# MalvinaNikandrou/mafed

Measured on AMD Instinct MI355X. Metric: train samples/sec VLPythia-410M+MAFED, 256img+32txt tok, bs=32, 1/2/4/8 GPU, higher is better.
Workload: dtype bf16; 1 GPU; VLPythia-410m + MAFED distill step (student fwd+bwd, frozen-teacher fwd, replay CE, 23-layer per-modality MSE, clip 2.0, AdamW), 256 img + 32 txt tokens; global_batch=32, per_gpu_batch=32, seq_len=288, parallelism=dp1, random_init_weights=True

## Files before the change

### mafed_amd/csrc/attn_mfma.hip

```cpp
#include <type_traits>

#include "attn.h"
#include "row8.h"

namespace mafed {

namespace {

typedef __attribute__((address_space(3))) bf16x4* lds_bf16x4_ptr;

template <int D>
__device__ __forceinline__ int swz(int row) {
  if (D == 64) return ((row >> 1) & 3) << 1;
  if (D == 128) return (row & 7) << 1;
  return ((row & 7) << 1) | ((row >> 3) & 1);
}
template <int D>
__device__ __forceinline__ int tile_off(int row, int chunk) {
  if (D == 64) return row * 128 + ((chunk ^ swz<64>(row)) << 4);
  if (D == 128) return row * 256 + ((chunk ^ swz<128>(row)) << 4);
  return row * 512 + ((chunk ^ (((row & 7) << 1) | ((row >> 3) & 1))) << 4);
}

__device__ __forceinline__ uint4 load_chunk_rot(const bf16_t* __restrict__ rowp, int chunk, int rot, const float* __restrict__ rc,
// ... 256 lines not shown
  const bf16_t* kb = qb + D;
  const bf16_t* vb = qb + 2 * D;
  const int q0 = qt * 64 + wave * 16;
  const int myq = q0 + (lane & 15);
  const int g = lane >> 4;

  bf16x8 qf[D / 32];
  load_col_frags<D, true>(qf, qb, rstride, q0, S, rot, rc, rs, lane);

  f32x4 o[D / 16];
#pragma unroll
  for (int i = 0; i < D / 16; ++i) o[i] = (f32x4){0.f, 0.f, 0.f, 0.f};
  float m = -INFINITY, l = 0.f;
  const float scale = rsqrtf((float)D);

  for (int kt = 0; kt <= qt; ++kt) {
    __syncthreads();
    stage_rows<D, 64, true>(kimg, kb, rstride, kt * 64, S, rot, rc, rs, tid);
    stage_rows<D, 64, false>(vimg, vb, rstride, kt * 64, S, rot, rc, rs, tid);
    __syncthreads();
    const bool need_mask = (kt == qt) || (kt * 64 + 63 >= P);
    fwd_tile_step<D>(kimg, vimg, qf, o, m, l, scale, need_mask, kt * 64, g, lane,
                     [&](int key) { return key > myq || !key_ok(am, b, key, P, T, S); });
  }
  l = col_sum(l);
  if (myq < S) {
    store_out<D>(out + ((int64_t)b * S + myq) * H * D + (int64_t)h * D, o, l, g);
    if (g == 0) lse[((int64_t)b * H + h) * S + myq] = m + logf(l);
  }
}

template <int D>
__global__ __launch_bounds__(256) void attn_suffix_mfma_kernel(const bf16_t* __restrict__ qkv_img, const int64_t* __restrict__ image_index,
                                                               const bf16_t* __restrict__ qkv_txt, SuffixShape sh, const float* __restrict__ rc,
                                                               const float* __restrict__ rs, const int64_t* __restrict__ am,
                                                               bf16_t* __restrict__ out) {
  extern __shared__ __attribute__((aligned(16))) char lds[];
  char* kimg = lds;
  char* vimg = lds + 64 * D * 2;
  const int tid = threadIdx.x, lane = tid & 63;
  const int wave = __builtin_amdgcn_readfirstlane(tid >> 6);
  const int P = sh.P, T = sh.T, S = sh.P + sh.T, H = sh.H, rot = sh.rot;
  const int qt = blockIdx.x, h = blockIdx.y, b = blockIdx.z;
  const int64_t rstride = (int64_t)H * 3 * D;
  const bf16_t* ib = qkv_img + (suffix_image(image_index, b, sh.N) * P * H + h) * 3 * D;
  const bf16_t* tb = qkv_txt + ((int64_t)b * T * H + h) * 3 * D;
  const int q0 = qt * 64 + wave * 16;
  const int myq = q0 + (lane & 15), mypos = P + myq;
  const int g = lane >> 4;
  const bool active = q0 < T;

  bf16x8 qf[D / 32];
#pragma unroll
  for (int ks = 0; ks < D / 32; ++ks)
    qf[ks] = __builtin_bit_cast(bf16x8, load_chunk_rot(tb + (int64_t)myq * rstride, ks * 4 + g, rot, rc, rs, mypos, myq < T));

  f32x4 o[D / 16];
#pragma unroll
  for (int i = 0; i < D / 16; ++i) o[i] = (f32x4){0.f, 0.f, 0.f, 0.f};
  float m = -INFINITY, l = 0.f;
  const float scale = rsqrtf((float)D);
  const int last_q = min(qt * 64 + 63, T - 1);
  const int nkt = (P + last_q) / 64 + 1;

  for (int kt = 0; kt < nkt; ++kt) {
    __syncthreads();
    const auto row = [&](int gr) { return StageRow{gr < P ? ib + (int64_t)gr * rstride : tb + (int64_t)(gr - P) * rstride, gr, gr < S}; };
    stage_rows_by<D, true>(kimg, tid, kt * 64, D, rot, rc, rs, row);
    stage_rows_by<D, false>(vimg, tid, kt * 64, 2 * D, rot, rc, rs, row);
    __syncthreads();
    if (!active || kt * 64 > P + q0 + 15) continue;
    const bool need_mask = kt * 64 + 63 >= P;
    fwd_tile_step<D>(kimg, vimg, qf, o, m, l, scale, need_mask, kt * 64, g, lane,
                     [&](int key) { return key > mypos || !key_ok(am, b, key, P, T, S); });
  }
  l = col_sum(l);
  if (myq < T) store_out<D>(out + ((int64_t)b * T + myq) * H * D + (int64_t)h * D, o, l, g);
}

template <int D>
__global__ __launch_bounds__(256) void attn_cand_mfma_kernel(const bf16_t* __restrict__ qkv_pre, const bf16_t* __restrict__ qkv_cand, CandShape sh,
                                                             const float* __restrict__ rc, const float* __restrict__ rs,
                                                             const int64_t* __restrict__ am, bf16_t* __restrict__ out) {
  extern __shared__ __attribute__((aligned(16))) char lds[];
  char* kimg = lds;
  char* vimg = lds + 64 * D * 2;
  const int tid = threadIdx.x, lane = tid & 63;
  const int wave = __builtin_amdgcn_readfirstlane(tid >> 6);
  const int S0 = sh.S0, T = sh.T, P = sh.S0 - sh.T, A = sh.A, CA = sh.C * sh.A, H = sh.H, rot = sh.rot;
  const int qt = blockIdx.x, h = blockIdx.y, b = blockIdx.z;
  const int64_t rstride = (int64_t)H * 3 * D;
  const bf16_t* pb = qkv_pre + ((int64_t)b * S0 * H + h) * 3 * D;
  const bf16_t* cb = qkv_cand + ((int64_t)b * CA * H + h) * 3 * D;
  const int q0 = qt * 64 + wave * 16;
  const int myq = q0 + (lane & 15);
  const int mystart = myq / A * A;
  const int g = lane >> 4;
  const bool active = q0 < CA;

  bf16x8 qf[D / 32];
#pragma unroll
  for (int ks = 0; ks < D / 32; ++ks)
    qf[ks] = __builtin_bit_cast(bf16x8, load_chunk_rot(cb + (int64_t)myq * rstride, ks * 4 + g, rot, rc, rs, S0 + myq % A, myq < CA));

  f32x4 o[D / 16];
#pragma unroll
  for (int i = 0; i < D / 16; ++i) o[i] = (f32x4){0.f, 0.f, 0.f, 0.f};
  float m = -INFINITY, l = 0.f;
  const float scale = rsqrtf((float)D);
  const int nkp = (S0 + 63) / 64;
  const int k0 = qt * 64 / A * A;
  const int nkc = (min(qt * 64 + 63, CA - 1) - k0) / 64 + 1;
  const int wlo = q0 / A * A, whi = q0 + 15;

  for (int kt = 0; kt < nkp + nkc; ++kt) {
    const bool pre = kt < nkp;
    const int t0 = pre ? kt * 64 : k0 + (kt - nkp) * 64;
    __syncthreads();
    if (pre) {
      stage_rows<D, 64, true>(kimg, pb + D, rstride, t0, S0, rot, rc, rs, tid);
      stage_rows<D, 64, false>(vimg, pb + 2 * D, rstride, t0, S0, rot, rc, rs, tid);
    } else {
      const auto row = [&](int gr) { return StageRow{cb + (int64_t)gr * rstride, S0 + gr % A, gr < CA}; };
      stage_rows_by<D, true>(kimg, tid, t0, D, rot, rc, rs, row);
      stage_rows_by<D, false>(vimg, tid, t0, 2 * D, rot, rc, rs, row);
    }
    __syncthreads();
    if (!active || (!pre && (t0 > whi || t0 + 63 < wlo))) continue;
    const bool need_mask = !pre || t0 + 63 >= P;
    fwd_tile_step<D>(kimg, vimg, qf, o, m, l, scale, need_mask, t0, g, lane,
                     [&](int key) { return pre ? !key_ok(am, b, key, P, T, S0) : (key < mystart || key > myq); });
  }
  l = col_sum(l);
  if (myq < CA) store_out<D>(out + ((int64_t)b * CA + myq) * H * D + (int64_t)h * D, o, l, g);
}

template <int D>
__global__ __launch_bounds__(256) void attn_bwd_dq_mfma_kernel(const bf16_t* __restrict__ qkv, const bf16_t* __restrict__ out,
                                                               const bf16_t* __restrict__ dout, const float* __restrict__ lse, AttnShape sh,
                                                               const float* __restrict__ rc, const float* __restrict__ rs,
                                                               const int64_t* __restrict__ am, bf16_t* __restrict__ dqkv,
                                                               float* __restrict__ delta) {
  extern __shared__ __attribute__((aligned(16))) char lds[];
  char* kimg = lds;
  char* vimg = lds + 64 * D * 2;
  const int tid = threadIdx.x, lane = tid & 63, wave = tid >> 6;
  const int S = sh.S, H = sh.H, rot = sh.rot, P = sh.P, T = sh.T;
  const int qt = (int)gridDim.x - 1 - (int)blockIdx.x, h = blockIdx.y, b = blockIdx.z;
  const int64_t rstride = (int64_t)H * 3 * D;
  const bf16_t* qb = qkv + ((int64_t)b * S * H + h) * 3 * D;
  const bf16_t* kb = qb + D;
  const bf16_t* vb = qb + 2 * D;
  const int q0 = qt * 64 + wave * 16;
  const int myq = q0 + (lane & 15);
  const int g = lane >> 4;
  const int64_t ostride = (int64_t)H * D;
  const bf16_t* ob = out + (int64_t)b * S * ostride + (int64_t)h * D;
  const bf16_t* dob = dout + (int64_t)b * S * ostride + (int64_t)h * D;

  bf16x8 qf[D / 32], dof[D / 32];
  load_col_frags<D, true>(qf, qb, rstride, q0, S, rot, rc, rs, lane);
  load_col_frags<D, false>(dof, dob, ostride, q0, S, 0, rc, rs, lane);
  float dl = 0.f;
  {
    bf16x8 of[D / 32];
    load_col_frags<D, false>(of, ob, ostride, q0, S, 0, rc, rs, lane);
#pragma unroll
    for (int ks = 0; ks < D / 32; ++ks)
#pragma unroll
      for (int e = 0; e < 8; ++e) dl += (float)dof[ks][e] * (float)of[ks][e];
    dl = col_sum(dl);
  }
  float L = 0.f;
  if (myq < S) {
    L = lse[((int64_t)b * H + h) * S + myq];
    if (g == 0) delta[((int64_t)b * H + h) * S + myq] = dl;
  }
  f32x4 dq[D / 16];
#pragma unroll
  for (int i = 0; i < D / 16; ++i) dq[i] = (f32x4){0.f, 0.f, 0.f, 0.f};
  const float scale = rsqrtf((float)D);

  for (int kt = 0; kt <= qt; ++kt) {
    __syncthreads();
    stage_rows<D, 64, true>(kimg, kb, rstride, kt * 64, S, rot, rc, rs, tid);
    stage_rows<D, 64, false>(vimg, vb, rstride, kt * 64, S, rot, rc, rs, tid);
    __syncthreads();
    const bool need_mask = (kt == qt) || (kt * 64 + 63 >= P);
    f32x4 ds[4];
#pragma unroll
    for (int j = 0; j < 4; ++j) {
      f32x4 s = (f32x4){0.f, 0.f, 0.f, 0.f}, dp = (f32x4){0.f, 0.f, 0.f, 0.f};
#pragma unroll
      for (int ks = 0; ks < D / 32; ++ks) {
        s = __builtin_amdgcn_mfma_f32_16x16x32_bf16(frag_row<D>(kimg, j, ks, lane), qf[ks], s, 0, 0, 0);
        dp = __builtin_amdgcn_mfma_f32_16x16x32_bf16(frag_row<D>(vimg, j, ks, lane), dof[ks], dp, 0, 0, 0);
      }
#pragma unroll
      for (int r = 0; r < 4; ++r) {
        float p = __expf(s[r] * scale - L);
        if (need_mask) {
          const int key = kt * 64 + j * 16 + 4 * g + r;
          if (key > myq || !key_ok(am, b, key, P, T, S)) p = 0.f;
        }
        ds[j][r] = p * (dp[r] - dl) * scale;
      }
    }
    const bf16x8 d0 = pack_acc(ds[0], ds[1]), d1 = pack_acc(ds[2], ds[3]);
#pragma unroll
    for (int dt = 0; dt < D / 16; ++dt) {
      dq[dt] = __builtin_amdgcn_mfma_f32_16x16x32_bf16(frag_tr<D>(kimg, dt, 0, lane), d0, dq[dt], 0, 0, 0);
      dq[dt] = __builtin_amdgcn_mfma_f32_16x16x32_bf16(frag_tr<D>(kimg, dt, 1, lane), d1, dq[dt], 0, 0, 0);
    }
  }
  bf16_t* dqp = dqkv + ((int64_t)b * S * H + h) * 3 * D + (int64_t)myq * rstride;
  store_grad_unrot<D>(dqp, dq, rot, rc, rs, myq, lane, myq < S);
}

template <int D>
__global__ __launch_bounds__(256) void attn_bwd_dkv_mfma_kernel(const bf16_t* __restrict__ qkv, const bf16_t* __restrict__ dout,
                                                                const float* __restrict__ lse, const float* __restrict__ delta, AttnShape sh,
                                                                const float* __restrict__ rc, const float* __restrict__ rs,
                                                                const int64_t* __restrict__ am, bf16_t* __restrict__ dqkv) {
  extern __shared__ __attribute__((aligned(16))) char lds[];
  char* qimg = lds;
  char* doimg = lds + 64 * D * 2;
  float* Ls = reinterpret_cast<float*>(lds + 2 * 64 * D * 2);
  float* dls = Ls + 64;
  const int tid = threadIdx.x, lane = tid & 63, wave = tid >> 6;
  const int S = sh.S, H = sh.H, rot = sh.rot, P = sh.P, T = sh.T;
  const int kt = blockIdx.x, h = blockIdx.y, b = blockIdx.z;
  const int nqt = (S + 63) / 64;
  const int64_t rstride = (int64_t)H * 3 * D;
  const bf16_t* qb = qkv + ((int64_t)b * S * H + h) * 3 * D;
  const bf16_t* kb = qb + D;
  const bf16_t* vb = qb + 2 * D;
  const int64_t ostride = (int64_t)H * D;
  const bf16_t* dob = dout + (int64_t)b * S * ostride + (int64_t)h * D;
  const int k0 = kt * 64 + wave * 16;
  const int mykey = k0 + (lane & 15);
  const int g = lane >> 4;
  const bool mykey_ok = key_ok(am, b, mykey, P, T, S);

  bf16x8 kf[D / 32], vf[D / 32];
  load_col_frags<D, true>(kf, kb, rstride, k0, S, rot, rc, rs, lane);
  load_col_frags<D, false>(vf, vb, rstride, k0, S, 0, rc, rs, lane);
  f32x4 dk[D / 16], dv[D / 16];
#pragma unroll
  for (int i = 0; i < D / 16; ++i) { dk[i] = (f32x4){0.f, 0.f, 0.f, 0.f}; dv[i] = (f32x4){0.f, 0.f, 0.f, 0.f}; }
  const float scale = rsqrtf((float)D);
  const int64_t lbase = ((int64_t)b * H + h) * S;

  for (int qt = kt; qt < nqt; ++qt) {
    __syncthreads();
    stage_rows<D, 64, true>(qimg, qb, rstride, qt * 64, S, rot, rc, rs, tid);
    stage_rows<D, 64, false>(doimg, dob, ostride, qt * 64, S, 0, rc, rs, tid);
    if (tid < 64) {
      const int q = qt * 64 + tid;
      Ls[tid] = q < S ? lse[lbase + q] : 0.f;
      dls[tid] = q < S ? delta[lbase + q] : 0.f;
    }
    __syncthreads();
    f32x4 p[4], ds[4];
#pragma unroll
    for (int j = 0; j < 4; ++j) {
      f32x4 s = (f32x4){0.f, 0.f, 0.f, 0.f}, dp = (f32x4){0.f, 0.f, 0.f, 0.f};
#pragma unroll
      for (int ks = 0; ks < D / 32; ++ks) {
        s = __builtin_amdgcn_mfma_f32_16x16x32_bf16(frag_row<D>(qimg, j, ks, lane), kf[ks], s, 0, 0, 0);
        dp = __builtin_amdgcn_mfma_f32_16x16x32_bf16(frag_row<D>(doimg, j, ks, lane), vf[ks], dp, 0, 0, 0);
      }
      const float4 Lq = *reinterpret_cast<const float4*>(Ls + j * 16 + 4 * g);
      const float4 Dq = *reinterpret_cast<const float4*>(dls + j * 16 + 4 * g);
      const float La[4] = {Lq.x, Lq.y, Lq.z, Lq.w}, Da[4] = {Dq.x, Dq.y, Dq.z, Dq.w};
#pragma unroll
      for (int r = 0; r < 4; ++r) {
        const int q = qt * 64 + j * 16 + 4 * g + r;
        float pv = __expf(s[r] * scale - La[r]);
        if (!mykey_ok || mykey > q || q >= S) pv = 0.f;
        p[j][r] = pv;
        ds[j][r] = pv * (dp[r] - Da[r]) * scale;
      }
    }
    const bf16x8 p0 = pack_acc(p[0], p[1]), p1 = pack_acc(p[2], p[3]);
    const bf16x8 d0 = pack_acc(ds[0], ds[1]), d1 = pack_acc(ds[2], ds[3]);
#pragma unroll
    for (int dt = 0; dt < D / 16; ++dt) {
      dv[dt] = __builtin_amdgcn_mfma_f32_16x16x32_bf16(frag_tr<D>(doimg, dt, 0, lane), p0, dv[dt], 0, 0, 0);
      dv[dt] = __builtin_amdgcn_mfma_f32_16x16x32_bf16(frag_tr<D>(doimg, dt, 1, lane), p1, dv[dt], 0, 0, 0);
      dk[dt] = __builtin_amdgcn_mfma_f32_16x16x32_bf16(frag_tr<D>(qimg, dt, 0, lane), d0, dk[dt], 0, 0, 0);
      dk[dt] = __builtin_amdgcn_mfma_f32_16x16x32_bf16(frag_tr<D>(qimg, dt, 1, lane), d1, dk[dt], 0, 0, 0);
    }
  }
  bf16_t* dkp = dqkv + ((int64_t)b * S * H + h) * 3 * D + (int64_t)mykey * rstride + D;
  store_grad_unrot<D>(dkp, dk, rot, rc, rs, mykey, lane, mykey < S);
  if (mykey < S) {
    bf16_t* dvp = dkp + D;
#pragma unroll
    for (int dt = 0; dt < D / 16; ++dt) store4(dvp + dt * 16 + 4 * g, make_float4(dv[dt][0], dv[dt][1], dv[dt][2], dv[dt][3]));
  }
}

typedef __attribute__((address_space(3))) void* lds_void_ptr;
typedef const __attribute__((address_space(1))) void* glb_void_ptr;
typedef unsigned u32x2 __attribute__((ext_vector_type(2)));

__device__ __forceinline__ float col_max_sw(float v) {
  u32x2 r = __builtin_amdgcn_permlane32_swap(__float_as_uint(v), __float_as_uint(v), false, false);
  v = fmaxf(__uint_as_float(r[0]), __uint_as_float(r[1]));
  r = __builtin_amdgcn_permlane16_swap(__float_as_uint(v), __float_as_uint(v), false, false);
  return fmaxf(__uint_as_float(r[0]), __uint_as_float(r[1]));
}
__device__ __forceinline__ float col_sum_sw(float v) {
  u32x2 r = __builtin_amdgcn_permlane32_swap(__float_as_uint(v), __float_as_uint(v), false, false);
  v = __uint_as_float(r[0]) + __uint_as_float(r[1]);
  r = __builtin_amdgcn_permlane16_swap(__float_as_uint(v), __float_as_uint(v), false, false);
  return __uint_as_float(r[0]) + __uint_as_float(r[1]);
}

template <int D, int NW = 4>
__device__ __forceinline__ void dma_rows(char* __restrict__ img, const bf16_t* __restrict__ base, int64_t rstride, int nrows, int S, int wave,
                                         int lane) {
  constexpr int RPP = 1024 / (2 * D);
  const int npieces = nrows / RPP;
  for (int j = wave; j < npieces; j += NW) {
    int row, logical;
    if (D == 64) {
      row = j * 8 + (lane >> 3);
      logical = (lane & 7) ^ swz<64>(row);
    } else {
      row = j * 4 + (lane >> 4);
      logical = (lane & 15) ^ swz<128>(row);
    }
    const int srow = row < S ? row : S - 1;
    __builtin_amdgcn_global_load_lds((glb_void_ptr)(base + (int64_t)srow * rstride + logical * 8), (lds_void_ptr)(img + j * 1024), 16, 0, 0);
  }
}

struct RotPre {
  float4 c0, c1, s0, s1;
};
__device__ __forceinline__ void rot_pre_load(RotPre& r, int it, int hc, int rot, const float* __restrict__ rc, const float* __restrict__ rs) {
  const int row = it / hc, c = it - row * hc;
  const float* cp = rc + (int64_t)row * (rot >> 1) + c * 8;
  const float* sp = rs + (int64_t)row * (rot >> 1) + c * 8;
  r.c0 = load4(cp); r.c1 = load4(cp + 4); r.s0 = load4(sp); r.s1 = load4(sp + 4);
}
template <int D>
__device__ __forceinline__ void rot_apply(char* __restrict__ img, int it, int hc, const RotPre& r) {
  const int row = it / hc, c = it - row * hc;
  uint4* p1 = reinterpret_cast<uint4*>(img + tile_off<D>(row, c));
  uint4* p2 = reinterpret_cast<uint4*>(img + tile_off<D>(row, c + hc));
  float x1[8], x2[8], o1[8], o2[8];
  unpack8(*p1, x1);
  unpack8(*p2, x2);
  const float cs[8] = {r.c0.x, r.c0.y, r.c0.z, r.c0.w, r.c1.x, r.c1.y, r.c1.z, r.c1.w};
  const float sn[8] = {r.s0.x, r.s0.y, r.s0.z, r.s0.w, r.s1.x, r.s1.y, r.s1.z, r.s1.w};
#pragma unroll
  for (int e = 0; e < 8; ++e) {
    o1[e] = x1[e] * cs[e] - x2[e] * sn[e];
    o2[e] = x2[e] * cs[e] + x1[e] * sn[e];
  }
  *p1 = pack8(o1);
  *p2 = pack8(o2);
}
template <int D, int NT = 256>
__device__ __forceinline__ void rot_fix_rows(char* __restrict__ img, int items, int hc, int rot, const float* __restrict__ rc,
                                             const float* __restrict__ rs, const RotPre (&pre)[2], int tid) {
#pragma unroll
  for (int u = 0; u < 2; ++u)
    if (tid + NT * u < items) rot_apply<D>(img, tid + NT * u, hc, pre[u]);
  for (int it = tid + 2 * NT; it < items; it += NT) {
    RotPre r;
    rot_pre_load(r, it, hc, rot, rc, rs);
    rot_apply<D>(img, it, hc, r);
  }
}

__device__ __forceinline__ float row16_sum(float v) {
  v += __builtin_bit_cast(float, __builtin_amdgcn_update_dpp(0, __builtin_bit_cast(int, v), 0xB1, 0xF, 0xF, true));
  v += __builtin_bit_cast(float, __builtin_amdgcn_update_dpp(0, __builtin_bit_cast(int, v), 0x4E, 0xF, 0xF, true));
  v += __builtin_bit_cast(float, __builtin_amdgcn_update_dpp(0, __builtin_bit_cast(int, v), 0x141, 0xF, 0xF, true));
  v += __builtin_bit_cast(float, __builtin_amdgcn_update_dpp(0, __builtin_bit_cast(int, v), 0x140, 0xF, 0xF, true));
  return v;
}

__device__ __forceinline__ void wait_vm0() { asm volatile("s_waitcnt vmcnt(0)" ::: "memory"); }

__device__ __forceinline__ int snake4(int w, int t) { return t * 4 + ((t & 1) ? 3 - w : w); }
template <int NW>
__device__ __forceinline__ int snake(int w, int t) { return t * NW + ((t & 1) ? NW - 1 - w : w); }

#define MAFED_LOG2E 1.4426950408889634f
#define MAFED_LN2 0.6931471805599453f

template <int D>
constexpr int attn_fwd_waves() { return D == 64 ? 8 : 4; }

template <int D, bool CAUSAL = true>
__global__ __launch_bounds__(attn_fwd_waves<D>() * 64, (D == 64 ? 2 : 1) * attn_fwd_waves<D>() / 4) void attn_fwd_res_kernel(const bf16_t* __restrict__ qkv, AttnShape sh, const float* __restrict__ rc,
                                                           const float* __restrict__ rs, const int64_t* __restrict__ am,
                                                           bf16_t* __restrict__ out, float* __restrict__ lse) {
  extern __shared__ __attribute__((aligned(16))) char lds[];
  constexpr int NW = attn_fwd_waves<D>(), NTH = NW * 64;
  const int tid = threadIdx.x, lane = tid & 63;
  const int wave = __builtin_amdgcn_readfirstlane(tid >> 6);
  const int S = sh.S, H = sh.H, rot = sh.rot, P = sh.P, T = sh.T;
  const int h = blockIdx.x, b = blockIdx.y;
  const int nrows = (S + 31) / 32 * 32;
  char* kimg = lds;
  char* vimg = lds + nrows * D * 2;
  float* kbias = reinterpret_cast<float*>(lds + 2 * nrows * D * 2);
  const int64_t rstride = (int64_t)H * 3 * D;
  const bf16_t* qb = qkv + ((int64_t)b * S * H + h) * 3 * D;
  const bf16_t* kb = qb + D;
  const bf16_t* vb = qb + 2 * D;
  const int nslices = (S + 15) / 16;
  const int hc = rot >> 4, items = S * hc;
#if defined(MAFED_ATTN_ABL) && MAFED_ATTN_ABL == 3
  if (tid == 0) out[((int64_t)b * S) * H * D + (int64_t)h * D] = 0;
  return;
#endif
  dma_rows<D, NW>(kimg, kb, rstride, nrows, S, wave, lane);
#if !defined(MAFED_ATTN_ABL) || MAFED_ATTN_ABL != 4
  dma_rows<D, NW>(vimg, vb, rstride, nrows, S, wave, lane);
#endif
  RotPre pre[2];
#pragma unroll
  for (int u = 0; u < 2; ++u)
    if (tid + NTH * u < items) rot_pre_load(pre[u], tid + NTH * u, hc, rot, rc, rs);
  for (int k = tid; k < nrows; k += NTH) kbias[k] = key_ok(am, b, k, P, T, S) ? 0.f : -INFINITY;
  ColRaw<D> qraw;
  {
    const int s0 = nslices - 1 - snake<NW>(wave, 0);
    if (s0 >= 0) col_raw_issue<D, true>(qraw, qb, rstride, s0 * 16, S, rot, rc, rs, lane);
  }
  wait_vm0();
  __syncthreads();
  rot_fix_rows<D, NTH>(kimg, items, hc, rot, rc, rs, pre, tid);
  __syncthreads();
#if defined(MAFED_ATTN_ABL) && (MAFED_ATTN_ABL == 1 || MAFED_ATTN_ABL == 4)
  if (tid < 64) out[((int64_t)b * S + tid) * H * D + (int64_t)h * D] = *reinterpret_cast<const bf16_t*>(kimg + tid * 1024) + *reinterpret_cast<const bf16_t*>(vimg + tid * 1024);
  return;
#endif
  const int g = lane >> 4;
  const float scale2 = rsqrtf((float)D) * MAFED_LOG2E;
  const bf16x8 ones = __builtin_bit_cast(bf16x8, make_uint4(0x3f803f80u, 0x3f803f80u, 0x3f803f80u, 0x3f803f80u));
  for (int t = 0;; ++t) {
    const int slice = nslices - 1 - snake<NW>(wave, t);
    if (slice < 0) break;
    const int q0 = slice * 16;
    const int myq = q0 + (lane & 15);
    bf16x8 qf[D / 32];
    col_raw_finish<D, true>(qf, qraw, q0, S, rot, lane);
    {
      const int nxt = nslices - 1 - snake<NW>(wave, t + 1);
      if (nxt >= 0) col_raw_issue<D, true>(qraw, qb, rstride, nxt * 16, S, rot, rc, rs, lane);
    }
    f32x4 o[D / 16];
#pragma unroll
    for (int i = 0; i < D / 16; ++i) o[i] = (f32x4){0.f, 0.f, 0.f, 0.f};
    float m = -INFINITY;
    f32x4 lsum = (f32x4){0.f, 0.f, 0.f, 0.f};
    const int last_kt = CAUSAL ? (q0 + 15) / 64 : (S - 1) / 64;
    auto tile = [&](const int kt, const int nj, auto mask_tag) {
      constexpr bool MASK = decltype(mask_tag)::value;
      f32x4 s[4];
#pragma unroll
      for (int j = 0; j < 4; ++j) {
        s[j] = (f32x4){0.f, 0.f, 0.f, 0.f};
        if (!MASK || j < nj) {
#pragma unroll
          for (int ks = 0; ks < D / 32; ++ks)
            s[j] = __builtin_amdgcn_mfma_f32_16x16x32_bf16(frag_row<D>(kimg, kt * 4 + j, ks, lane), qf[ks], s[j], 0, 0, 0);
        }
      }
      float tmax = -INFINITY;
      if (MASK) {
#pragma unroll
        for (int j = 0; j < 4; ++j) {
          if (j < nj) {
            const float4 kb4 = *reinterpret_cast<const float4*>(kbias + kt * 64 + j * 16 + 4 * g);
            const float kbv[4] = {kb4.x, kb4.y, kb4.z, kb4.w};
#pragma unroll
            for (int r = 0; r < 4; ++r) {
              const int key = kt * 64 + j * 16 + 4 * g + r;
              float v = s[j][r] * scale2 + kbv[r];
              if (CAUSAL) v = key > myq ? -INFINITY : v;
              s[j][r] = v;
              tmax = fmaxf(tmax, v);
            }
          } else {
            s[j] = (f32x4){-INFINITY, -INFINITY, -INFINITY, -INFINITY};
          }
        }
      } else {
#pragma unroll
        for (int j = 0; j < 4; ++j)
#pragma unroll
          for (int r = 0; r < 4; ++r) tmax = fmaxf(tmax, s[j][r]);
        tmax *= scale2;
      }
      tmax = col_max_sw(tmax);
      if (__builtin_amdgcn_ballot_w64(tmax - m > 8.0f) != 0) {
        const float mn = fmaxf(m, tmax);
        const float alpha = __builtin_amdgcn_exp2f(m - mn);
        m = mn;
        lsum *= alpha;
#pragma unroll
        for (int i = 0; i < D / 16; ++i) o[i] *= alpha;
      }
#pragma unroll
      for (int j = 0; j < 4; ++j)
#pragma unroll
        for (int r = 0; r < 4; ++r) s[j][r] = __builtin_amdgcn_exp2f(MASK ? s[j][r] - m : fmaf(s[j][r], scale2, -m));
      const bf16x8 p0 = pack_acc(s[0], s[1]);
      lsum = __builtin_amdgcn_mfma_f32_16x16x32_bf16(ones, p0, lsum, 0, 0, 0);
#pragma unroll
      for (int dt = 0; dt < D / 16; ++dt) o[dt] = __builtin_amdgcn_mfma_f32_16x16x32_bf16(frag_tr<D>(vimg, dt, kt * 2, lane), p0, o[dt], 0, 0, 0);
      if (!MASK || nj > 2) {
        const bf16x8 p1 = pack_acc(s[2], s[3]);
        lsum = __builtin_amdgcn_mfma_f32_16x16x32_bf16(ones, p1, lsum, 0, 0, 0);
#pragma unroll
        for (int dt = 0; dt < D / 16; ++dt)
          o[dt] = __builtin_amdgcn_mfma_f32_16x16x32_bf16(frag_tr<D>(vimg, dt, kt * 2 + 1, lane), p1, o[dt], 0, 0, 0);
      }
    };
    const int kt_plain = CAUSAL ? (last_kt < P / 64 ? last_kt : P / 64) : (P / 64 <= last_kt ? P / 64 : last_kt + 1);
    const int klast = CAUSAL ? q0 + 15 : S - 1;
    for (int kt = 0; kt < kt_plain; ++kt) tile(kt, 4, std::false_type{});
    for (int kt = kt_plain; kt <= last_kt; ++kt) tile(kt, kt == last_kt ? ((klast - kt * 64) >> 4) + 1 : 4, std::true_type{});
    const float l = lsum[0];
    if (myq < S) {
      const float inv = 1.0f / l;
      bf16_t* op = out + ((int64_t)b * S + myq) * H * D + (int64_t)h * D;
#pragma unroll
      for (int dt = 0; dt < D / 16; ++dt)
        store4(op + dt * 16 + 4 * g, make_float4(o[dt][0] * inv, o[dt][1] * inv, o[dt][2] * inv, o[dt][3] * inv));
      if (g == 0) lse[((int64_t)b * H + h) * S + myq] = m * MAFED_LN2 + logf(l);
    }
  }
}

template <int D, int NW = 4>
__global__ __launch_bounds__(NW * 64, (D == 64 ? 2 : 1) * NW / 4) void attn_bwd_dq_res_kernel(const bf16_t* __restrict__ qkv, const bf16_t* __restrict__ out,
                                                              const bf16_t* __restrict__ dout, const float* __restrict__ lse, AttnShape sh,
                                                              const float* __restrict__ rc, const float* __restrict__ rs,
                                                              const int64_t* __restrict__ am, bf16_t* __restrict__ dqkv,
                                                              float* __restrict__ delta, float* __restrict__ bsum) {
  extern __shared__ __attribute__((aligned(16))) char lds[];
  constexpr int NTH = NW * 64;
  const int tid = threadIdx.x, lane = tid & 63;
  const int wave = __builtin_amdgcn_readfirstlane(tid >> 6);
  const int S = sh.S, H = sh.H, rot = sh.rot, P = sh.P, T = sh.T;
  const int h = blockIdx.x, b = blockIdx.y;
  const int nrows = (S + 31) / 32 * 32;
  char* kimg = lds;
  char* vimg = lds + nrows * D * 2;
  float* kbias = reinterpret_cast<float*>(lds + 2 * nrows * D * 2);
  float* red = kbias + 2 * nrows;
  if (bsum && tid < D) red[tid] = 0.f;
  const int64_t rstride = (int64_t)H * 3 * D;
  const bf16_t* qb = qkv + ((int64_t)b * S * H + h) * 3 * D;
  const bf16_t* kb = qb + D;
  const bf16_t* vb = qb + 2 * D;
  const int64_t ostride = (int64_t)H * D;
  const bf16_t* ob = out + (int64_t)b * S * ostride + (int64_t)h * D;
  const bf16_t* dob = dout + (int64_t)b * S * ostride + (int64_t)h * D;
  const float* Lrow = lse + ((int64_t)b * H + h) * S;
  const int nslices = (S + 15) / 16;
  const int hc = rot >> 4, items = S * hc;
  dma_rows<D, NW>(kimg, kb, rstride, nrows, S, wave, lane);
  dma_rows<D, NW>(vimg, vb, rstride, nrows, S, wave, lane);
  RotPre pre[2];
#pragma unroll
  for (int u = 0; u < 2; ++u)
    if (tid + NTH * u < items) rot_pre_load(pre[u], tid + NTH * u, hc, rot, rc, rs);
  for (int k = tid; k < nrows; k += NTH) kbias[k] = key_ok(am, b, k, P, T, S) ? 0.f : -INFINITY;
  constexpr bool PREFETCH = NW == 4;
  ColRaw<D> qraw, doraw, oraw;
  float Lnext = 0.f;
  if (PREFETCH) {
    const int s0 = nslices - 1 - snake<NW>(wave, 0);
    if (s0 >= 0) {
      col_raw_issue<D, true>(qraw, qb, rstride, s0 * 16, S, rot, rc, rs, lane);
      col_raw_issue<D, false>(doraw, dob, ostride, s0 * 16, S, 0, rc, rs, lane);
      col_raw_issue<D, false>(oraw, ob, ostride, s0 * 16, S, 0, rc, rs, lane);
      const int q = s0 * 16 + (lane & 15);
      Lnext = q < S ? Lrow[q] : 0.f;
    }
  }
  wait_vm0();
  __syncthreads();
  rot_fix_rows<D, NTH>(kimg, items, hc, rot, rc, rs, pre, tid);
  __syncthreads();
  const int g = lane >> 4;
  const float scale = rsqrtf((float)D);
  const float scale2 = scale * MAFED_LOG2E;
  for (int t = 0;; ++t) {
    const int slice = nslices - 1 - snake<NW>(wave, t);
    if (slice < 0) break;
    const int q0 = slice * 16;
    const int myq = q0 + (lane & 15);
    if (!PREFETCH) {
      col_raw_issue<D, true>(qraw, qb, rstride, q0, S, rot, rc, rs, lane);
      col_raw_issue<D, false>(doraw, dob, ostride, q0, S, 0, rc, rs, lane);
      col_raw_issue<D, false>(oraw, ob, ostride, q0, S, 0, rc, rs, lane);
      Lnext = myq < S ? Lrow[myq] : 0.f;
    }
    bf16x8 qf[D / 32], dof[D / 32];
    col_raw_finish<D, true>(qf, qraw, q0, S, rot, lane);
    col_raw_finish<D, false>(dof, doraw, q0, S, 0, lane);
    const float L2 = Lnext * MAFED_LOG2E;
    float dl = 0.f;
    {
      bf16x8 of[D / 32];
      col_raw_finish<D, false>(of, oraw, q0, S, 0, lane);
      const int nxt = nslices - 1 - snake<NW>(wave, t + 1);
      if (PREFETCH && nxt >= 0) {
        col_raw_issue<D, true>(qraw, qb, rstride, nxt * 16, S, rot, rc, rs, lane);
        col_raw_issue<D, false>(doraw, dob, ostride, nxt * 16, S, 0, rc, rs, lane);
        col_raw_issue<D, false>(oraw, ob, ostride, nxt * 16, S, 0, rc, rs, lane);
        const int q = nxt * 16 + (lane & 15);
        Lnext = q < S ? Lrow[q] : 0.f;
      }
#pragma unroll
      for (int ks = 0; ks < D / 32; ++ks)
#pragma unroll
        for (int e = 0; e < 8; ++e) dl += (float)dof[ks][e] * (float)of[ks][e];
      dl = col_sum_sw(dl);
    }
    if (myq < S && g == 0) delta[((int64_t)b * H + h) * S + myq] = dl;
    f32x4 dq[D / 16];
#pragma unroll
    for (int i = 0; i < D / 16; ++i) dq[i] = (f32x4){0.f, 0.f, 0.f, 0.f};
    const int last_kt = (q0 + 15) / 64;
    auto tile = [&](const int kt, const int nj, auto mask_tag) {
      constexpr bool MASK = decltype(mask_tag)::value;
      f32x4 ds[4];
#pragma unroll
      for (int j = 0; j < 4; ++j) {
        ds[j] = (f32x4){0.f, 0.f, 0.f, 0.f};
        if (!MASK || j < nj) {
          f32x4 s = (f32x4){0.f, 0.f, 0.f, 0.f}, dp = (f32x4){0.f, 0.f, 0.f, 0.f};
#pragma unroll
          for (int ks = 0; ks < D / 32; ++ks) {
            s = __builtin_amdgcn_mfma_f32_16x16x32_bf16(frag_row<D>(kimg, kt * 4 + j, ks, lane), qf[ks], s, 0, 0, 0);
            dp = __builtin_amdgcn_mfma_f32_16x16x32_bf16(frag_row<D>(vimg, kt * 4 + j, ks, lane), dof[ks], dp, 0, 0, 0);
          }
          if (MASK) {
            const float4 kb4 = *reinterpret_cast<const float4*>(kbias + kt * 64 + j * 16 + 4 * g);
            const float kbv[4] = {kb4.x, kb4.y, kb4.z, kb4.w};
#pragma unroll
            for (int r = 0; r < 4; ++r) {
              const int key = kt * 64 + j * 16 + 4 * g + r;
              float x = s[r] * scale2 - L2 + kbv[r];
              x = key > myq ? -INFINITY : x;
              ds[j][r] = __builtin_amdgcn_exp2f(x) * (dp[r] - dl) * scale;
            }
          } else {
#pragma unroll
            for (int r = 0; r < 4; ++r) ds[j][r] = __builtin_amdgcn_exp2f(s[r] * scale2 - L2) * (dp[r] - dl) * scale;
          }
        }
      }
      const bf16x8 d0 = pack_acc(ds[0], ds[1]);
#pragma unroll
      for (int dt = 0; dt < D / 16; ++dt) dq[dt] = __builtin_amdgcn_mfma_f32_16x16x32_bf16(frag_tr<D>(kimg, dt, kt * 2, lane), d0, dq[dt], 0, 0, 0);
      if (!MASK || nj > 2) {
        const bf16x8 d1 = pack_acc(ds[2], ds[3]);
#pragma unroll
        for (int dt = 0; dt < D / 16; ++dt)
          dq[dt] = __builtin_amdgcn_mfma_f32_16x16x32_bf16(frag_tr<D>(kimg, dt, kt * 2 + 1, lane), d1, dq[dt], 0, 0, 0);
      }
    };
    const int kt_plain = last_kt < P / 64 ? last_kt : P / 64;
    for (int kt = 0; kt < kt_plain; ++kt) tile(kt, 4, std::false_type{});
    for (int kt = kt_plain; kt <= last_kt; ++kt) tile(kt, kt == last_kt ? ((q0 + 15 - kt * 64) >> 4) + 1 : 4, std::true_type{});
    bf16_t* dqp = dqkv + ((int64_t)b * S * H + h) * 3 * D + (int64_t)myq * rstride;
    store_grad_unrot<D>(dqp, dq, rot, rc, rs, myq, lane, myq < S);
    if (bsum) {
#pragma unroll
      for (int dt = 0; dt < D / 16; ++dt)
#pragma unroll
        for (int r = 0; r < 4; ++r) {
          const float v = row16_sum(myq < S ? dq[dt][r] : 0.f);
          if ((lane & 15) == 0) atomicAdd(red + dt * 16 + 4 * g + r, v);
        }
    }
  }
  if (bsum) {
    __syncthreads();
    if (tid < D) atomicAdd(bsum + (int64_t)h * 3 * D + tid, red[tid]);
  }
}

template <int D, int NW = 4>
__global__ __launch_bounds__(NW * 64, (D == 64 ? 2 : 1) * NW / 4) void attn_bwd_dkv_res_kernel(const bf16_t* __restrict__ qkv, const bf16_t* __restrict__ dout,
                                                               const float* __restrict__ lse, const float* __restrict__ delta, AttnShape sh,
                                                               const float* __restrict__ rc, const float* __restrict__ rs,
                                                               const int64_t* __restrict__ am, bf16_t* __restrict__ dqkv,
                                                               float* __restrict__ bsum) {
  extern __shared__ __attribute__((aligned(16))) char lds[];
  constexpr int NTH = NW * 64;
  const int tid = threadIdx.x, lane = tid & 63;
  const int wave = __builtin_amdgcn_readfirstlane(tid >> 6);
  const int S = sh.S, H = sh.H, rot = sh.rot, P = sh.P, T = sh.T;
  const int h = blockIdx.x, b = blockIdx.y;
  const int nrows = (S + 31) / 32 * 32;
  char* qimg = lds;
  char* doimg = lds + nrows * D * 2;
  float* L2s = reinterpret_cast<float*>(lds + 2 * nrows * D * 2);
  float* Ds = L2s + nrows;
  float* red = Ds + nrows;
  if (bsum && tid < 2 * D) red[tid] = 0.f;
  const int64_t rstride = (int64_t)H * 3 * D;
  const bf16_t* qb = qkv + ((int64_t)b * S * H + h) * 3 * D;
  const bf16_t* kb = qb + D;
  const bf16_t* vb = qb + 2 * D;
  const int64_t ostride = (int64_t)H * D;
  const bf16_t* dob = dout + (int64_t)b * S * ostride + (int64_t)h * D;
  const float* Lrow = lse + ((int64_t)b * H + h) * S;
  const float* Drow = delta + ((int64_t)b * H + h) * S;
  const int nslices = (S + 15) / 16;
  const int hc = rot >> 4, items = S * hc;
  dma_rows<D, NW>(qimg, qb, rstride, nrows, S, wave, lane);
  dma_rows<D, NW>(doimg, dob, ostride, nrows, S, wave, lane);
  RotPre pre[2];
#pragma unroll
  for (int u = 0; u < 2; ++u)
    if (tid + NTH * u < items) rot_pre_load(pre[u], tid + NTH * u, hc, rot, rc, rs);
  for (int q = tid; q < nrows; q += NTH) {
    L2s[q] = q < S ? Lrow[q] * MAFED_LOG2E : INFINITY;
    Ds[q] = q < S ? Drow[q] : 0.f;
  }
  ColRaw<D> kraw, vraw;
  {
    const int s0 = snake<NW>(wave, 0);
    if (s0 < nslices) {
      col_raw_issue<D, true>(kraw, kb, rstride, s0 * 16, S, rot, rc, rs, lane);
      col_raw_issue<D, false>(vraw, vb, rstride, s0 * 16, S, 0, rc, rs, lane);
    }
  }
  wait_vm0();
  __syncthreads();
  rot_fix_rows<D, NTH>(qimg, items, hc, rot, rc, rs, pre, tid);
  __syncthreads();
  const int g = lane >> 4;
  const float scale = rsqrtf((float)D);
  const float scale2 = scale * MAFED_LOG2E;
  const int nqt = (nrows + 63) / 64;
  for (int t = 0;; ++t) {
    const int slice = snake<NW>(wave, t);
    if (slice >= nslices) break;
    const int k0 = slice * 16;
    const int mykey = k0 + (lane & 15);
    const int mykey_eff = key_ok(am, b, mykey, P, T, S) ? mykey : 0x7fffffff;
    bf16x8 kf[D / 32], vf[D / 32];
    col_raw_finish<D, true>(kf, kraw, k0, S, rot, lane);
    col_raw_finish<D, false>(vf, vraw, k0, S, 0, lane);
    {
      const int nxt = snake<NW>(wave, t + 1);
      if (nxt < nslices) {
        col_raw_issue<D, true>(kraw, kb, rstride, nxt * 16, S, rot, rc, rs, lane);
        col_raw_issue<D, false>(vraw, vb, rstride, nxt * 16, S, 0, rc, rs, lane);
      }
    }
    f32x4 dk[D / 16], dv[D / 16];
#pragma unroll
    for (int i = 0; i < D / 16; ++i) { dk[i] = (f32x4){0.f, 0.f, 0.f, 0.f}; dv[i] = (f32x4){0.f, 0.f, 0.f, 0.f}; }
    const int qt0 = k0 / 64;
    const bool text_keys = k0 + 15 >= P;
    auto tile = [&](const int qt, const int jlo, const int jhi, auto edge_tag) {
      constexpr bool EDGE = decltype(edge_tag)::value;
      f32x4 p[4], ds[4];
#pragma unroll
      for (int j = 0; j < 4; ++j) {
        p[j] = (f32x4){0.f, 0.f, 0.f, 0.f};
        ds[j] = (f32x4){0.f, 0.f, 0.f, 0.f};
        if (!EDGE || (j >= jlo && j < jhi)) {
          f32x4 s = (f32x4){0.f, 0.f, 0.f, 0.f}, dp = (f32x4){0.f, 0.f, 0.f, 0.f};
#pragma unroll
          for (int ks = 0; ks < D / 32; ++ks) {
            s = __builtin_amdgcn_mfma_f32_16x16x32_bf16(frag_row<D>(qimg, qt * 4 + j, ks, lane), kf[ks], s, 0, 0, 0);
            dp = __builtin_amdgcn_mfma_f32_16x16x32_bf16(frag_row<D>(doimg, qt * 4 + j, ks, lane), vf[ks], dp, 0, 0, 0);
          }
          const float4 L4 = *reinterpret_cast<const float4*>(L2s + qt * 64 + j * 16 + 4 * g);
          const float4 D4 = *reinterpret_cast<const float4*>(Ds + qt * 64 + j * 16 + 4 * g);
          const float Lv[4] = {L4.x, L4.y, L4.z, L4.w}, Dv[4] = {D4.x, D4.y, D4.z, D4.w};
#pragma unroll
          for (int r = 0; r < 4; ++r) {
            float x = s[r] * scale2 - Lv[r];
            if (EDGE) {
              const int q = qt * 64 + j * 16 + 4 * g + r;
              x = mykey_eff > q ? -INFINITY : x;
            }
            const float pv = __builtin_amdgcn_exp2f(x);
            p[j][r] = pv;
            ds[j][r] = pv * (dp[r] - Dv[r]) * scale;
          }
        }
      }
      if (!EDGE || jlo < 2) {
        const bf16x8 p0 = pack_acc(p[0], p[1]), d0 = pack_acc(ds[0], ds[1]);
#pragma unroll
        for (int dt = 0; dt < D / 16; ++dt) {
          dv[dt] = __builtin_amdgcn_mfma_f32_16x16x32_bf16(frag_tr<D>(doimg, dt, qt * 2, lane), p0, dv[dt], 0, 0, 0);
          dk[dt] = __builtin_amdgcn_mfma_f32_16x16x32_bf16(frag_tr<D>(qimg, dt, qt * 2, lane), d0, dk[dt], 0, 0, 0);
        }
      }
      if (!EDGE || jhi > 2) {
        const bf16x8 p1 = pack_acc(p[2], p[3]), d1 = pack_acc(ds[2], ds[3]);
#pragma unroll
        for (int dt = 0; dt < D / 16; ++dt) {
          dv[dt] = __builtin_amdgcn_mfma_f32_16x16x32_bf16(frag_tr<D>(doimg, dt, qt * 2 + 1, lane), p1, dv[dt], 0, 0, 0);
          dk[dt] = __builtin_amdgcn_mfma_f32_16x16x32_bf16(frag_tr<D>(qimg, dt, qt * 2 + 1, lane), d1, dk[dt], 0, 0, 0);
        }
      }
    };
    const int nfull = nrows / 64;
    for (int qt = qt0; qt < nqt; ++qt) {
      const int jlo = qt == qt0 ? (k0 - qt * 64) >> 4 : 0;
      const int jhi = (nrows - qt * 64) >> 4 < 4 ? (nrows - qt * 64) >> 4 : 4;
      if (qt == qt0 || text_keys || qt >= nfull) tile(qt, jlo, jhi, std::true_type{});
      else tile(qt, 0, 4, std::false_type{});
    }
    bf16_t* dkp = dqkv + ((int64_t)b * S * H + h) * 3 * D + (int64_t)mykey * rstride + D;
    store_grad_unrot<D>(dkp, dk, rot, rc, rs, mykey, lane, mykey < S);
    if (mykey < S) {
      bf16_t* dvp = dkp + D;
#pragma unroll
      for (int dt = 0; dt < D / 16; ++dt) store4(dvp + dt * 16 + 4 * g, make_float4(dv[dt][0], dv[dt][1], dv[dt][2], dv[dt][3]));
    }
    if (bsum) {
#pragma unroll
      for (int dt = 0; dt < D / 16; ++dt)
#pragma unroll
        for (int r = 0; r < 4; ++r) {
          const float vk = row16_sum(mykey < S ? dk[dt][r] : 0.f), vv = row16_sum(mykey < S ? dv[dt][r] : 0.f);
          if ((lane & 15) == 0) {
            atomicAdd(red + dt * 16 + 4 * g + r, vk);
            atomicAdd(red + D + dt * 16 + 4 * g + r, vv);
          }
// ... 132 lines not shown
```

Baseline: 1014 samples/s.

## Defer V tile DMA to overlap with K rotary fix and first QK tile

The forward attention kernel now issues the V global-to-LDS copy after the K rotary fix-up instead of alongside K. It waits for V only inside the first key tile, after the QK scores and softmax for that tile are computed, so V loading overlaps with rotary work and the first score computation. Waves with no query slice still take part in the matching barriers at the end. The global_load_lds call is also replaced by inline assembly that sets M0 explicitly, and lane is laundered through an empty asm to steer codegen. This adds barrier-count coupling across waves and fragile inline asm.

```diff
diff --git a/mafed_amd/csrc/attn_mfma.hip b/mafed_amd/csrc/attn_mfma.hip
--- a/mafed_amd/csrc/attn_mfma.hip
+++ b/mafed_amd/csrc/attn_mfma.hip
@@ -582,7 +582,6 @@
 }
 
 typedef __attribute__((address_space(3))) void* lds_void_ptr;
-typedef const __attribute__((address_space(1))) void* glb_void_ptr;
 typedef unsigned u32x2 __attribute__((ext_vector_type(2)));
 
 __device__ __forceinline__ float col_max_sw(float v) {
@@ -603,6 +602,7 @@
                                          int lane) {
   constexpr int RPP = 1024 / (2 * D);
   const int npieces = nrows / RPP;
+  const uint32_t img0 = (uint32_t)(uintptr_t)(lds_void_ptr)img;
   for (int j = wave; j < npieces; j += NW) {
     int row, logical;
     if (D == 64) {
@@ -613,7 +613,12 @@
       logical = (lane & 15) ^ swz<128>(row);
     }
     const int srow = row < S ? row : S - 1;
-    __builtin_amdgcn_global_load_lds((glb_void_ptr)(base + (int64_t)srow * rstride + logical * 8), (lds_void_ptr)(img + j * 1024), 16, 0, 0);
+    const bf16_t* src = base + (int64_t)srow * rstride + logical * 8;
+    unsigned keep;
+    asm volatile("s_mov_b32 %0, m0\n\ts_mov_b32 m0, %2\n\ts_nop 0\n\tglobal_load_lds_dwordx4 %1, off\n\ts_mov_b32 m0, %0"
+                 : "=&s"(keep)
+                 : "v"(src), "s"(img0 + (uint32_t)j * 1024u)
+                 : "memory");
   }
 }
 
@@ -702,24 +707,27 @@
   return;
 #endif
   dma_rows<D, NW>(kimg, kb, rstride, nrows, S, wave, lane);
-#if !defined(MAFED_ATTN_ABL) || MAFED_ATTN_ABL != 4
-  dma_rows<D, NW>(vimg, vb, rstride, nrows, S, wave, lane);
-#endif
   RotPre pre[2];
 #pragma unroll
   for (int u = 0; u < 2; ++u)
     if (tid + NTH * u < items) rot_pre_load(pre[u], tid + NTH * u, hc, rot, rc, rs);
   for (int k = tid; k < nrows; k += NTH) kbias[k] = key_ok(am, b, k, P, T, S) ? 0.f : -INFINITY;
   ColRaw<D> qraw;
-  {
-    const int s0 = nslices - 1 - snake<NW>(wave, 0);
-    if (s0 >= 0) col_raw_issue<D, true>(qraw, qb, rstride, s0 * 16, S, rot, rc, rs, lane);
-  }
+  const int slice0 = nslices - 1 - snake<NW>(wave, 0);
+  if (slice0 >= 0) col_raw_issue<D, true>(qraw, qb, rstride, slice0 * 16, S, rot, rc, rs, lane);
   wait_vm0();
   __syncthreads();
   rot_fix_rows<D, NTH>(kimg, items, hc, rot, rc, rs, pre, tid);
+  auto request_v = [&]() {
+#if !defined(MAFED_ATTN_ABL) || MAFED_ATTN_ABL != 4
+    dma_rows<D, NW>(vimg, vb, rstride, nrows, S, wave, lane);
+#endif
+    __syncthreads();
+  };
+#if defined(MAFED_ATTN_ABL) && (MAFED_ATTN_ABL == 1 || MAFED_ATTN_ABL == 4)
+  request_v();
+  wait_vm0();
   __syncthreads();
-#if defined(MAFED_ATTN_ABL) && (MAFED_ATTN_ABL == 1 || MAFED_ATTN_ABL == 4)
   if (tid < 64) out[((int64_t)b * S + tid) * H * D + (int64_t)h * D] = *reinterpret_cast<const bf16_t*>(kimg + tid * 1024) + *reinterpret_cast<const bf16_t*>(vimg + tid * 1024);
   return;
 #endif
@@ -733,9 +741,12 @@
     const int myq = q0 + (lane & 15);
     bf16x8 qf[D / 32];
     col_raw_finish<D, true>(qf, qraw, q0, S, rot, lane);
+    if (t == 0) request_v();
     {
       const int nxt = nslices - 1 - snake<NW>(wave, t + 1);
-      if (nxt >= 0) col_raw_issue<D, true>(qraw, qb, rstride, nxt * 16, S, rot, rc, rs, lane);
+      int ln = lane;
+      asm volatile("" : "+v"(ln));
+      if (nxt >= 0) col_raw_issue<D, true>(qraw, qb, rstride, nxt * 16, S, rot, rc, rs, ln);
     }
     f32x4 o[D / 16];
 #pragma unroll
@@ -743,8 +754,8 @@
     float m = -INFINITY;
     f32x4 lsum = (f32x4){0.f, 0.f, 0.f, 0.f};
     const int last_kt = CAUSAL ? (q0 + 15) / 64 : (S - 1) / 64;
-    auto tile = [&](const int kt, const int nj, auto mask_tag) {
-      constexpr bool MASK = decltype(mask_tag)::value;
+    auto tile = [&](const int kt, const int nj, auto mask_tag, auto first_tag) {
+      constexpr bool MASK = decltype(mask_tag)::value, FIRST = decltype(first_tag)::value;
       f32x4 s[4];
 #pragma unroll
       for (int j = 0; j < 4; ++j) {
@@ -796,6 +807,10 @@
         for (int r = 0; r < 4; ++r) s[j][r] = __builtin_amdgcn_exp2f(MASK ? s[j][r] - m : fmaf(s[j][r], scale2, -m));
       const bf16x8 p0 = pack_acc(s[0], s[1]);
       lsum = __builtin_amdgcn_mfma_f32_16x16x32_bf16(ones, p0, lsum, 0, 0, 0);
+      if (FIRST) {
+        wait_vm0();
+        __syncthreads();
+      }
 #pragma unroll
       for (int dt = 0; dt < D / 16; ++dt) o[dt] = __builtin_amdgcn_mfma_f32_16x16x32_bf16(frag_tr<D>(vimg, dt, kt * 2, lane), p0, o[dt], 0, 0, 0);
       if (!MASK || nj > 2) {
@@ -808,8 +823,15 @@
     };
     const int kt_plain = CAUSAL ? (last_kt < P / 64 ? last_kt : P / 64) : (P / 64 <= last_kt ? P / 64 : last_kt + 1);
     const int klast = CAUSAL ? q0 + 15 : S - 1;
-    for (int kt = 0; kt < kt_plain; ++kt) tile(kt, 4, std::false_type{});
-    for (int kt = kt_plain; kt <= last_kt; ++kt) tile(kt, kt == last_kt ? ((klast - kt * 64) >> 4) + 1 : 4, std::true_type{});
+    const auto nj_of = [&](int kt) { return kt == last_kt ? ((klast - kt * 64) >> 4) + 1 : 4; };
+    int kt = 0;
+    if (t == 0) {
+      if (kt_plain > 0) tile(0, 4, std::false_type{}, std::true_type{});
+      else tile(0, nj_of(0), std::true_type{}, std::true_type{});
+      kt = 1;
+    }
+    for (; kt < kt_plain; ++kt) tile(kt, 4, std::false_type{}, std::false_type{});
+    for (kt = kt < kt_plain ? kt_plain : kt; kt <= last_kt; ++kt) tile(kt, nj_of(kt), std::true_type{}, std::false_type{});
     const float l = lsum[0];
     if (myq < S) {
       const float inv = 1.0f / l;
@@ -819,6 +841,11 @@
         store4(op + dt * 16 + 4 * g, make_float4(o[dt][0] * inv, o[dt][1] * inv, o[dt][2] * inv, o[dt][3] * inv));
       if (g == 0) lse[((int64_t)b * H + h) * S + myq] = m * MAFED_LN2 + logf(l);
     }
+  }
+  if (slice0 < 0) {
+    request_v();
+    wait_vm0();
+    __syncthreads();
   }
 }
 
```

New measurement: 1009 samples/s. No clear change (-0.5%).
